# ETH3D/badslam

Hardware: NVIDIA H100
Metric: surfel_keyframe_residuals_per_second_per_BA_iteration (higher is better)
Workload: dtype f32

## Files before the change

badslam_b200/csrc/handle.hpp:

```cpp
#pragma once

#include <cuda_runtime.h>

#include <algorithm>
#include <atomic>
#include <condition_variable>
#include <cstdio>
#include <cstdlib>
#include <map>
#include <mutex>
#include <string>
#include <thread>
#include <vector>

#include "../../include/badba.h"
#include "host_math.hpp"
#include "kernels.cuh"
#include "odometry.cuh"

namespace bba {

template <class R, auto Free>
struct Owned {
  R r{};
// ... 115 lines not shown
  float depth_a = 0.f;
  int cf_w = 0, cf_h = 0;
  int sm_count = 132;
  std::mutex error_mu;
  std::map<std::thread::id, std::string> errors;

  float* surfels = nullptr;
  size_t surfel_pitch_bytes = 0;
  uint32_t surfels_size = 0;
  uint8_t* active = nullptr;
  bba::DeviceBuffer<float> owned_surfels;
  size_t owned_surfel_pitch = 0;
  bba::DeviceBuffer<uint8_t> owned_active;

  bba::DeviceBuffer<float> d_cfactor;
  std::vector<bba::Keyframe> keyframes;
  bba::DeviceBuffer<bba::KfDevice> d_kfs;

  struct Staging {
    bba::PinnedBuffer<bba::KfDevice> h_kfs;
    bba::Event event;
    bool pending = false;
    bba::LumaStaging luma;
    bba::PitchedBuffer color;
    bba::Texture scratch;
  } staging;

  struct PoseStep {
    bba::DeviceBuffer<bba::KfDevice> d_work_records;
    bba::DeviceBuffer<float> d_pose_est;
    bba::DeviceBuffer<double> d_acc;
    bba::DeviceBuffer<unsigned long long> d_stage_counts;
    bba::DeviceBuffer<int> d_work[2];
    bba::DeviceBuffer<int> d_count;
    bba::DeviceBuffer<int> d_iterations;
    bba::DeviceBuffer<int> d_converged;
    bba::DeviceBuffer<double> d_first_stats;
    bba::DeviceBuffer<unsigned long long> d_totals;
    bba::DeviceBuffer<unsigned int> d_queue;
    bba::MappedBuffer<int> flag;
    volatile int* h_flag = nullptr;
    int* d_flag = nullptr;
    bba::PinnedBuffer<float> h_pose_est;
    bba::PinnedBuffer<int> h_work;
    bba::PinnedBuffer<int> h_iterations;
    bba::PinnedBuffer<int> h_converged;
    bba::PinnedBuffer<double> h_first_stats;
    bba::PinnedBuffer<unsigned long long> h_totals;
    struct Order {
      bba::DeviceBuffer<uint32_t> words;
      bba::DeviceBuffer<unsigned char> temp;
      bba::DeviceBuffer<float> stream;
      bba::DeviceBuffer<float> boxes;
      bba::SpatialOrderBuffers view{};
      uint32_t capacity = 0;
    } order;
    uint32_t order_n = 0;
    bool order_stale = true;
  } pose;

  struct Geometry {
    bba::DeviceBuffer<int> d_list;
    bba::PinnedBuffer<int> h_list;
    bba::DeviceBuffer<unsigned int> d_queue;
    bba::DeviceBuffer<unsigned int> d_tile_epoch;
    const uint32_t* perm = nullptr;
    bba::DeviceBuffer<float> d_intr;
    bba::DeviceBuffer<double> d_intr_sums;
    bba::DeviceBuffer<int> d_all_list;
    bba::PinnedBuffer<double> h_intr_sums;
    bba::PinnedBuffer<float> h_intr_x1;
  } geo;

  struct Lifecycle {
    bba::DeviceBuffer<unsigned int> d_sup;
    bba::DeviceBuffer<unsigned int> d_cell_bits;
    bba::DeviceBuffer<unsigned int> d_flags;
    bba::DeviceBuffer<unsigned int> d_scan_out;
    bba::DeviceBuffer<unsigned int> d_scan_sums;
    bba::DeviceBuffer<bba::CovisEntry> d_covis;
    bba::PinnedBuffer<bba::CovisEntry> h_covis;
    bba::DeviceBuffer<bba::KfRadius> d_kf_radius;
    bba::PinnedBuffer<bba::KfRadius> h_kf_radius;
    bba::DeviceBuffer<unsigned int> d_deleted_count;
    bba::PinnedBuffer<unsigned int> h_deleted_count;
    bba::DeviceBuffer<unsigned int> d_compact_sums;
  } life;
  int last_ba_iteration_count = -1;

  struct Pcg {
    bba::DeviceBuffer<float> d_vec[5];
    bba::DeviceBuffer<double> d_scalars;
    bba::PinnedBuffer<double> h_scalars;
    bba::PinnedBuffer<float> h_delta;
  } pcg;

  struct Exchange {
    bba_collective_fn collective = nullptr;
    void* collective_user = nullptr;
    bba::DeviceBuffer<float> d_exchange;
    bba::DeviceBuffer<float> d_pose_pack;
    bba::PinnedBuffer<float> h_pose_pack;
    bba::DeviceBuffer<int> d_local_ids;
    bba::DeviceBuffer<float> d_count_xchg;
    bba::PinnedBuffer<float> h_count_xchg;
    bba::DeviceBuffer<float> d_barrier;
// ... 139 lines not shown
```

badslam_b200/csrc/kernels.cu:

```cuda
#include "persistent.cuh"

#include <cuda.h>

#include <algorithm>

namespace bba {


__device__ __forceinline__ uint32_t SmemAddr(const void* p) { return static_cast<uint32_t>(__cvta_generic_to_shared(p)); }

__device__ __forceinline__ void MbarInit(uint64_t* bar, uint32_t count) {
  asm volatile("mbarrier.init.shared::cta.b64 [%0], %1;" ::"r"(SmemAddr(bar)), "r"(count));
}
__device__ __forceinline__ void FenceBarrierInit() { asm volatile("fence.mbarrier_init.release.cluster;" ::: "memory"); }
__device__ __forceinline__ void MbarArriveExpectTx(uint64_t* bar, uint32_t bytes) {
  asm volatile("mbarrier.arrive.expect_tx.shared::cta.b64 _, [%0], %1;" ::"r"(SmemAddr(bar)), "r"(bytes) : "memory");
}
__device__ __forceinline__ void MbarArrive(uint64_t* bar) {
  asm volatile("mbarrier.arrive.shared::cta.b64 _, [%0];" ::"r"(SmemAddr(bar)) : "memory");
}
__device__ __forceinline__ void MbarWait(uint64_t* bar, uint32_t parity) {
  asm volatile(
      "{\n"
      ".reg .pred p;\n"
      "WAIT_LOOP:\n"
      "mbarrier.try_wait.parity.shared::cta.b64 p, [%0], %1;\n"
      "@p bra.uni WAIT_DONE;\n"
      "bra.uni WAIT_LOOP;\n"
      "WAIT_DONE:\n"
      "}\n" ::"r"(SmemAddr(bar)),
      "r"(parity)
      : "memory");
}
__device__ __forceinline__ bool MbarTest(uint64_t* bar, uint32_t parity) {
  uint32_t done;
  asm volatile(
      "{\n"
      ".reg .pred p;\n"
      "mbarrier.test_wait.parity.shared::cta.b64 p, [%1], %2;\n"
      "selp.u32 %0, 1, 0, p;\n"
      "}\n"
      : "=r"(done)
      : "r"(SmemAddr(bar)), "r"(parity)
      : "memory");
  return done != 0;
}
__device__ __forceinline__ void BulkCopyG2S(void* smem_dst, const void* gmem_src, uint32_t bytes, uint64_t* bar) {
  asm volatile("cp.async.bulk.shared::cluster.global.mbarrier::complete_tx::bytes [%0], [%1], %2, [%3];" ::"r"(SmemAddr(smem_dst)),
               "l"(gmem_src), "r"(bytes), "r"(SmemAddr(bar))
               : "memory");
}


__device__ __forceinline__ cudaTextureObject_t UniformTexture(cudaTextureObject_t tex) {
  const unsigned long long t = tex;
  const unsigned lo = __shfl_sync(0xffffffffu, static_cast<unsigned>(t), 0);
  const unsigned hi = __shfl_sync(0xffffffffu, static_cast<unsigned>(t >> 32), 0);
  return (static_cast<unsigned long long>(hi) << 32) | lo;
}

constexpr int kPoseMinCtas = 2;
constexpr int kPoseChunkShift = 8;
constexpr int kPoseThreads = 256;
constexpr int kPoseUnroll = 1;
constexpr int kPoseStagedRows = 7;
constexpr int kPoseStagedRowsPre = 14;
static_assert(kPoseStagedRowsPre == kPoseStreamRows, "the PRE instantiations stage every row of the pose stream");
constexpr int kPoseGroup = 8;

__device__ __forceinline__ bool CornersOutsideView(const CameraParams& cam, const float* __restrict__ T, float px, float py, float pz) {
  float v[3], a[3];
#pragma unroll
  for (int r = 0; r < 3; ++r) {
    v[r] = T[4 * r] * px + T[4 * r + 1] * py + T[4 * r + 2] * pz + T[4 * r + 3];
    a[r] = fabsf(T[4 * r] * px) + fabsf(T[4 * r + 1] * py) + fabsf(T[4 * r + 2] * pz) + fabsf(T[4 * r + 3]);
  }
  constexpr float e = 1e-5f;
  const float l_x = cam.cx + 1.f, r_x = cam.cx - static_cast<float>(cam.w) - 1.f;
  const float l_y = cam.cy + 1.f, r_y = cam.cy - static_cast<float>(cam.h) - 1.f;
  unsigned out = (v[2] < -e * a[2]) ? 1u : 0u;
  out |= (cam.fx * v[0] + l_x * v[2] < -e * (cam.fx * a[0] + fabsf(l_x) * a[2])) ? 2u : 0u;
  out |= (cam.fx * v[0] + r_x * v[2] > e * (cam.fx * a[0] + fabsf(r_x) * a[2])) ? 4u : 0u;
  out |= (cam.fy * v[1] + l_y * v[2] < -e * (cam.fy * a[1] + fabsf(l_y) * a[2])) ? 8u : 0u;
  out |= (cam.fy * v[1] + r_y * v[2] > e * (cam.fy * a[1] + fabsf(r_y) * a[2])) ? 16u : 0u;
  if (!(cam.fx > 0.f && cam.fy > 0.f)) out &= 1u;
  return __reduce_and_sync(0xffffffffu, out) != 0u;
}
__device__ __forceinline__ bool BoxOutsideView(const CameraParams& cam, const float* __restrict__ T, const float* box, int lane) {
  const int c = lane & 7;
  return CornersOutsideView(cam, T, box[(c & 1) ? 4 : 0], box[(c & 2) ? 5 : 1], box[(c & 4) ? 6 : 2]);
}

constexpr int kPoseProducerWarps = 8;
constexpr int kPoseConsumerWarps = 4;
constexpr int kPoseWsThreads = 32 * (kPoseProducerWarps + kPoseConsumerWarps);
constexpr int kPoseProducerRegs = 72;
constexpr int kPoseConsumerRegs = 96;
static_assert(kPoseProducerWarps * kPoseProducerRegs + kPoseConsumerWarps * kPoseConsumerRegs ==
                  (kPoseProducerWarps + kPoseConsumerWarps) * 80, "register split");
constexpr int kPoseRecFields = 16;
constexpr int kPoseRingSlots = 2;
constexpr int kPoseBatchFloats = kPoseRecFields * 32;
constexpr size_t kPoseRingBytes = sizeof(float) * kPoseBatchFloats * kPoseRingSlots * kPoseProducerWarps;

template <int N>
__device__ __forceinline__ void SetMaxRegsDec() { asm volatile("setmaxnreg.dec.sync.aligned.u32 %0;\n" ::"n"(N)); }
template <int N>
__device__ __forceinline__ void SetMaxRegsInc() { asm volatile("setmaxnreg.inc.sync.aligned.u32 %0;\n" ::"n"(N)); }

template <bool STATS>
__device__ __forceinline__ void AccumulatePair(const CameraParams& cam, const Assoc& r, const DescEval& e, bool photo,
                                               float (&acc)[kPoseAccSize]) {
  acc[27] += 1.f;
  if (cam.use_depth) {
    float inv_stddev;
    Vec3 up;
    const float raw = DepthResidual(cam, r, &inv_stddev, &up);
    float J[6];
    DepthPoseJacobian(r, inv_stddev, up, J);
    AccumulateHb(acc, J, raw, DepthWeight(raw));
    if (STATS) acc[29] += DepthCost(raw);
  }
  if (cam.use_desc && photo) {
    acc[28] += 1.f;
    float J[6];
    DescPoseJacobian(cam, r.lp, e.gx1, e.gy1, J);
    AccumulateHb(acc, J, e.r1, DescWeight(e.r1));
    DescPoseJacobian(cam, r.lp, e.gx2, e.gy2, J);
    AccumulateHb(acc, J, e.r2, DescWeight(e.r2));
    if (STATS) {
      acc[30] += DescCost(e.r1);
      acc[31] += DescCost(e.r2);
    }
  }
}

template <bool STATS>
__device__ __forceinline__ void AccumulateRecord(const CameraParams& cam, const float* rec, float (&acc)[kPoseAccSize]) {
  Assoc r;
  r.lp = V3(rec[0 * 32], rec[1 * 32], rec[2 * 32]);
  r.ln = V3(rec[3 * 32], rec[4 * 32], rec[5 * 32]);
  r.d = rec[6 * 32];
  r.nx = rec[7 * 32];
  r.ny = rec[8 * 32];
  DescEval e;
  e.r1 = rec[9 * 32];
  e.r2 = rec[10 * 32];
  e.gx1 = rec[11 * 32];
  e.gy1 = rec[12 * 32];
  e.gx2 = rec[13 * 32];
  e.gy2 = rec[14 * 32];
  AccumulatePair<STATS>(cam, r, e, rec[15 * 32] != 0.f, acc);
}

template <int TILE, bool STATS, bool PRE>
__global__ void __launch_bounds__(PRE ? kPoseWsThreads : kPoseThreads, kPoseMinCtas)
    PoseAccumulateKernel(const __grid_constant__ PoseAccumulateArgs args) {
  constexpr int kRows = PRE ? kPoseStagedRowsPre : kPoseStagedRows;
  extern __shared__ __align__(128) unsigned char smem_raw[];
  float* stage_base = reinterpret_cast<float*>(smem_raw);
  float* rings = stage_base + 2 * kRows * TILE;
  __shared__ __align__(16) KfDevice s_kf[2][kPoseGroup];
  __shared__ __align__(16) float s_box[2][PRE ? TILE / kSpatialChunk : 1][8];
  __shared__ __align__(8) uint64_t full_bar[2];
  __shared__ unsigned int s_item[2];
  __shared__ int s_sub[2];
  __shared__ __align__(8) uint64_t batch_full[PRE ? kPoseProducerWarps : 1][kPoseRingSlots];
  __shared__ __align__(8) uint64_t batch_empty[PRE ? kPoseProducerWarps : 1][kPoseRingSlots];
  __shared__ int3 batch_hdr[PRE ? kPoseProducerWarps : 1][kPoseRingSlots];

  const int n_work = __ldg(args.work_count);
  if (n_work <= 0) return;

  const int tid = threadIdx.x;
  const int lane = tid & 31;
  const int warp = tid >> 5;
  const uint32_t n_tiles = (args.n + TILE - 1) / TILE;
  const uint32_t n_groups = (n_work + kPoseGroup - 1) / kPoseGroup;
  const uint32_t n_items = n_groups * n_tiles;
  constexpr int kTileShift = (TILE == 1024) ? 10 : (TILE == 512) ? 9 : 8;

  const CameraParams& cam = args.cam;
  constexpr int kRowIds[kPoseStagedRows] = {kRowX, kRowY, kRowZ, kRowNormal, kRowRadiusSq, kRowD1, kRowD2};

  auto issue_tile = [&](uint32_t item, int s) {
    const uint32_t group = item / n_tiles, tile = item - group * n_tiles;
    const uint32_t base = tile * TILE;
    const uint32_t cnt = min(static_cast<uint32_t>(TILE), args.n - base);
    const uint32_t bytes = ((cnt * 4u + 15u) / 16u) * 16u;
    const uint32_t kf_bytes = static_cast<uint32_t>(sizeof(KfDevice)) * min(kPoseGroup, n_work - static_cast<int>(group) * kPoseGroup);
    const uint32_t box_bytes = PRE ? (cnt + kSpatialChunk - 1) / kSpatialChunk * 8 * sizeof(float) : 0u;
    MbarArriveExpectTx(&full_bar[s], bytes * kRows + kf_bytes + box_bytes);
    BulkCopyG2S(&s_kf[s][0], args.work_records + static_cast<size_t>(group) * kPoseGroup, kf_bytes, &full_bar[s]);
    if (PRE) {
      BulkCopyG2S(&s_box[s][0][0], args.boxes + static_cast<size_t>(base / kSpatialChunk) * 8, box_bytes, &full_bar[s]);
#pragma unroll
      for (int r = 0; r < kPoseStreamRows; ++r)
        BulkCopyG2S(stage_base + (s * kRows + r) * TILE, args.stream + static_cast<size_t>(r) * args.stream_pitch + base, bytes,
                    &full_bar[s]);
    } else {
#pragma unroll
      for (int r = 0; r < kPoseStagedRows; ++r) {
        BulkCopyG2S(stage_base + (s * kRows + r) * TILE,
                    args.surfels + static_cast<size_t>(kRowIds[r]) * args.pitch + base, bytes, &full_bar[s]);
      }
    }
  };

  __shared__ int s_done[2];
  constexpr int kWarps = PRE ? kPoseProducerWarps : kPoseThreads / 32;
  auto arm_stage = [&](int s) {
    s_sub[s] = 0;
    s_done[s] = 0;
    const unsigned int item = atomicAdd(args.queue, 1u);
    s_item[s] = item;
    if (item < n_items) issue_tile(item, s);
    else MbarArrive(&full_bar[s]);
  };
  if (tid == 0) {
    MbarInit(&full_bar[0], 1);
    MbarInit(&full_bar[1], 1);
    if (PRE) {
      for (int p = 0; p < kPoseProducerWarps; ++p)
        for (int b = 0; b < kPoseRingSlots; ++b) {
          MbarInit(&batch_full[p][b], 32);
          MbarInit(&batch_empty[p][b], 32);
        }
    }
    FenceBarrierInit();
    arm_stage(0);
    arm_stage(1);
  }
  __syncthreads();

  uint32_t batch_seq = 0;
  bool batch_owned = false;
  int batch_fill = 0;
  if constexpr (PRE) {
    if (warp >= kPoseProducerWarps) {
      SetMaxRegsInc<kPoseConsumerRegs>();
      const int c = warp - kPoseProducerWarps;
      float acc0[kPoseAccSize], acc1[kPoseAccSize];
#pragma unroll
      for (int i = 0; i < kPoseAccSize; ++i) acc0[i] = acc1[i] = 0.f;
      uint32_t seq0 = 0, seq1 = 0;
      bool done0 = false, done1 = false;
      auto consume = [&](int p, uint32_t& seq, bool& done, float (&acc)[kPoseAccSize]) {
        const int b = seq & 1;
        if (!__all_sync(0xffffffffu, MbarTest(&batch_full[p][b], (seq >> 1) & 1))) return false;
        const int3 h = batch_hdr[p][b];
        if (h.z < 0) {
          done = true;
          return true;
        }
        if (lane < h.x) AccumulateRecord<STATS>(args.cam, rings + (p * kPoseRingSlots + b) * kPoseBatchFloats + lane, acc);
        MbarArrive(&batch_empty[p][b]);
        ++seq;
        if (h.y) {
          const float total = WarpTransposeReduce(acc, lane);
          atomicAdd(args.acc + static_cast<size_t>(h.z) * kPoseAccSize + lane, static_cast<double>(total));
#pragma unroll
          for (int i = 0; i < kPoseAccSize; ++i) acc[i] = 0.f;
        }
        return true;
      };
      while (!(done0 && done1)) {
        bool progress = false;
        if (!done0) progress |= consume(c, seq0, done0, acc0);
        if (!done1) progress |= consume(c + kPoseConsumerWarps, seq1, done1, acc1);
        if (!progress) __nanosleep(32);
      }
      return;
    }
    SetMaxRegsDec<kPoseProducerRegs>();
  }
  float* my_ring = rings + warp * kPoseRingSlots * kPoseBatchFloats;
  auto acquire_slot = [&](uint32_t u) {
    MbarWait(&batch_empty[warp][u & 1], ((u >> 1) & 1) ^ 1);
  };
  auto commit_slot = [&](uint32_t u, int pairs, bool last, int kf) {
    if (lane == 0) batch_hdr[warp][u & 1] = make_int3(pairs, last ? 1 : 0, kf);
    MbarArrive(&batch_full[warp][u & 1]);
  };

  for (uint32_t it = 0;; ++it) {
    const int s = it & 1;
    MbarWait(&full_bar[s], (it >> 1) & 1);
    const unsigned int item = *reinterpret_cast<volatile unsigned int*>(&s_item[s]);
    if (item >= n_items) break;

    const float* sx = stage_base + (s * kRows + 0) * TILE;
    const float* sy = sx + TILE;
    const float* sz = sy + TILE;
    const float* sn = sz + TILE;
    const float* sr = sn + TILE;
    const float* sd1 = PRE ? sz + TILE : sr + TILE;
    const float* sd2 = sd1 + TILE;
    const float* sf = sd2 + TILE;
    const uint32_t group = item / n_tiles;
    const uint32_t tile = item - group * n_tiles;
    const uint32_t base = tile * TILE;
    const uint32_t cnt = min(static_cast<uint32_t>(TILE), args.n - base);
    const int kfs_in_group = min(kPoseGroup, n_work - static_cast<int>(group) * kPoseGroup);
    const int wanted_shift = n_work >= 4 ? kPoseChunkShift : 7;
    const int chunk_shift = wanted_shift < kTileShift ? wanted_shift : kTileShift;
    const uint32_t chunk_len = 1u << chunk_shift;
    const int chunks_per_tile = TILE >> chunk_shift;
    const int n_sub = kfs_in_group * chunks_per_tile;

    for (;;) {
      int sub = 0;
      if (lane == 0) sub = atomicAdd(&s_sub[s], 1);
      sub = __shfl_sync(0xffffffffu, sub, 0);
      if (sub >= n_sub) break;
      const int kf_local = sub / chunks_per_tile;
      const uint32_t j0 = static_cast<uint32_t>(sub - kf_local * chunks_per_tile) << chunk_shift;
      if (j0 >= cnt) continue;
      const uint32_t j1 = min(cnt, j0 + chunk_len);
      KfRegs K;
      const int kf = LoadKfShared(&s_kf[s][kf_local], &K);
      if (PRE && BoxOutsideView(cam, K.T, s_box[s][PRE ? j0 / kSpatialChunk : 0], lane)) continue;
      K.tex = UniformTexture(K.tex);

      float acc[kPoseAccSize];
#pragma unroll
      for (int i = 0; i < kPoseAccSize; ++i) acc[i] = 0.f;
      unsigned touched = 0;
      unsigned n_inimg = 0, n_depthok = 0;

#pragma unroll kPoseUnroll
      for (uint32_t j = j0 + lane; j < j0 + (j1 - j0 + 31u) / 32u * 32u; j += 32) {
        int st = 0;
        Assoc r;
        Vec3 gp, nrm;
        DescEval e;
        bool photo = false;
        if (j < j1) {
          gp = V3(sx[j], sy[j], sz[j]);
          if (ProjectIntoImage(cam, K.T, gp, &r)) {
            const PixelLoads l = LoadPixel(cam, K.depth, K.depth_pitch, K.normals, K.normals_pitch, r);
            nrm = PRE ? V3(sf[j], sf[TILE + j], sf[2 * TILE + j]) : UnpackNormal(__float_as_uint(sn[j]));
            if (cam.use_desc) {
              float ccx, ccy;
              photo = DepthToColor(cam, r.pxf, r.pyf, &ccx, &ccy);
              float t1x, t1y, t2x, t2y;
              if (PRE) {
                ProjectTangentPoints(cam, K.T, V3(sf[3 * TILE + j], sf[4 * TILE + j], sf[5 * TILE + j]),
                                     V3(sf[6 * TILE + j], sf[7 * TILE + j], sf[8 * TILE + j]), &t1x, &t1y, &t2x, &t2y);
              } else {
                TangentProjections(cam, K.T, gp, nrm, sr[j], &t1x, &t1y, &t2x, &t2y);
              }
              EvalDescriptor(K.tex, ccx, ccy, t1x, t1y, t2x, t2y, sd1[j], sd2[j], &e);
            }
            st = Associate(cam, K.T, nrm, l, &r);
          }
        }
        if (STATS) {
          n_inimg += st >= 1;
          n_depthok += st >= 2;
        }
        const unsigned assoc_mask = __ballot_sync(0xffffffffu, st == 3);
        if (assoc_mask == 0) continue;
        touched |= assoc_mask;
        if constexpr (PRE) {
          const int m = __popc(assoc_mask);
          const int pos = batch_fill + __popc(assoc_mask & ((1u << lane) - 1u));
          const bool spill = batch_fill + m > 32;
          if (!batch_owned) acquire_slot(batch_seq);
          batch_owned = true;
          if (spill) acquire_slot(batch_seq + 1);
          if (st == 3) {
            float* rec = my_ring + ((batch_seq + (pos >> 5)) & 1) * kPoseBatchFloats + (pos & 31);
            rec[0 * 32] = r.lp.x; rec[1 * 32] = r.lp.y; rec[2 * 32] = r.lp.z;
            rec[3 * 32] = r.ln.x; rec[4 * 32] = r.ln.y; rec[5 * 32] = r.ln.z;
// ... 10 lines not shown
            batch_fill += m;
          }
        } else if (st == 3) {
          AccumulatePair<STATS>(cam, r, e, photo, acc);
        }
      }

      if (PRE && touched) {
        commit_slot(batch_seq, batch_fill, true, kf);
        ++batch_seq;
        batch_owned = false;
        batch_fill = 0;
      } else if (touched) {
        const float total = WarpTransposeReduce(acc, lane);
        atomicAdd(args.acc + static_cast<size_t>(kf) * kPoseAccSize + lane, static_cast<double>(total));
      }
      if (STATS) {
        n_inimg = __reduce_add_sync(0xffffffffu, n_inimg);
        n_depthok = __reduce_add_sync(0xffffffffu, n_depthok);
      }
      if (STATS && lane == 0 && n_inimg) {
        atomicAdd(args.stage_counts + 2 * kf, static_cast<unsigned long long>(n_inimg));
        if (n_depthok) atomicAdd(args.stage_counts + 2 * kf + 1, static_cast<unsigned long long>(n_depthok));
      }
    }
    __syncwarp();
    if (lane == 0) {
      __threadfence_block();
      if (atomicAdd(&s_done[s], 1) == kWarps - 1) {
        __threadfence_block();
        arm_stage(s);
      }
    }
  }
  if (PRE) {
    if (!batch_owned) acquire_slot(batch_seq);
    commit_slot(batch_seq, 0, false, -1);
  }
}

__global__ void __launch_bounds__(128) PackWorkRecordsKernel(const KfDevice* __restrict__ kfs, const int* __restrict__ work_list,
                                                             const int* __restrict__ work_count, KfDevice* __restrict__ records) {
  const int n = __ldg(work_count);
  constexpr int kWords = sizeof(KfDevice) / 16;
  for (int i = blockIdx.x * blockDim.x + threadIdx.x; i < n * kWords; i += gridDim.x * blockDim.x) {
    const int rec = i / kWords, w = i - rec * kWords;
    const int kf = __ldg(work_list + rec);
    uint4 v = __ldg(reinterpret_cast<const uint4*>(kfs + kf) + w);
    if (w == kWords - 1) v.y = static_cast<unsigned int>(kf);
    reinterpret_cast<uint4*>(records + rec)[w] = v;
  }
}

template <int TILE, bool STATS, bool PRE>
static void LaunchPoseAccumulateT(const PoseAccumulateArgs& args, int sm_count, cudaStream_t stream) {
  const size_t smem = static_cast<size_t>(2) * (PRE ? kPoseStagedRowsPre : kPoseStagedRows) * TILE * sizeof(float) + (PRE ? kPoseRingBytes : 0);
  static bool configured = false;
  if (!configured) {
    cudaFuncSetAttribute(PoseAccumulateKernel<TILE, STATS, PRE>, cudaFuncAttributeMaxDynamicSharedMemorySize, static_cast<int>(smem));
    configured = true;
  }
  PoseAccumulateKernel<TILE, STATS, PRE><<<kPoseMinCtas * sm_count, PRE ? kPoseWsThreads : kPoseThreads, smem, stream>>>(args);
}

template <bool STATS>
static void LaunchPoseAccumulateS(const PoseAccumulateArgs& args, int sm_count, int variant, cudaStream_t stream) {
  if (variant == kPoseVariantAuto) {
    const uint64_t slots = static_cast<uint64_t>(kPoseMinCtas * sm_count) * 4;
    if (args.stream != nullptr) variant = args.n >= slots * 512 ? kPoseVariant512Pre : kPoseVariant256Pre;
    else variant = args.n >= slots * 1024 ? kPoseVariant1024 : args.n >= slots * 512 ? kPoseVariant512 : kPoseVariant256;
  }
  switch (variant) {
    case kPoseVariant256Pre: LaunchPoseAccumulateT<256, STATS, true>(args, sm_count, stream); break;
    case kPoseVariant512Pre: LaunchPoseAccumulateT<512, STATS, true>(args, sm_count, stream); break;
    case kPoseVariant256: LaunchPoseAccumulateT<256, STATS, false>(args, sm_count, stream); break;
    case kPoseVariant512: LaunchPoseAccumulateT<512, STATS, false>(args, sm_count, stream); break;
    case kPoseVariant1024: LaunchPoseAccumulateT<1024, STATS, false>(args, sm_count, stream); break;
  }
}

void LaunchPoseAccumulate(const PoseAccumulateArgs& args, int sm_count, bool with_stats, int max_work, cudaStream_t stream, int variant) {
  if (args.n == 0) return;
  PackWorkRecordsKernel<<<(max_work * 6 + 127) / 128, 128, 0, stream>>>(args.kfs, args.work_list, args.work_count, args.work_records);
  if (with_stats) LaunchPoseAccumulateS<true>(args, sm_count, variant, stream);
  else LaunchPoseAccumulateS<false>(args, sm_count, variant, stream);
}


constexpr int kGeoThreads = 256;
constexpr int kGeoGroup = 32;

__device__ __forceinline__ void StageGroupRecords(const KfDevice* __restrict__ kfs, const int* __restrict__ kf_list, int count,
                                                  KfDevice* dst, int lane) {
  constexpr int kWords = sizeof(KfDevice) / 16;
  __syncwarp();
  const int my_kf = lane < count ? __ldg(kf_list + lane) : 0;
#pragma unroll
  for (int w = 0; w < (kGeoGroup * kWords + 31) / 32; ++w) {
    const int idx = w * 32 + lane, rec = idx / kWords, part = idx - rec * kWords;
    const int kf = __shfl_sync(0xffffffffu, my_kf, rec & 31);
    if (rec < count) {
      uint4 v = __ldg(reinterpret_cast<const uint4*>(kfs + kf) + part);
      reinterpret_cast<uint4*>(dst + rec)[part] = v;
    }
  }
  __syncwarp();
}

__device__ __forceinline__ void WarpBoxCorner(const Vec3& p, bool in, int lane, float* cx, float* cy, float* cz) {
  const float c[3] = {p.x, p.y, p.z};
  float corner[3];
#pragma unroll
  for (int ax = 0; ax < 3; ++ax) {
    const bool f = in && isfinite(c[ax]);
    const unsigned int lo = __reduce_min_sync(0xffffffffu, f ? OrderedBits(c[ax]) : 0xffffffffu);
    const unsigned int hi = __reduce_max_sync(0xffffffffu, f ? OrderedBits(c[ax]) : 0u);
    corner[ax] = FromOrderedBits(((lane >> ax) & 1) ? hi : lo);
  }
  *cx = corner[0];
  *cy = corner[1];
  *cz = corner[2];
}

__device__ __forceinline__ void StoreSurfelRow(const GeometryArgs& a, int row, uint32_t i, float v) {
  StoreReplicas(a.surfels, a.peers.surfels, a.peers.count, static_cast<size_t>(row) * a.pitch + i, v);
}

template <bool DETERMINE, bool NORMALS>
__global__ void __launch_bounds__(kGeoThreads) ActivationNormalsKernel(const __grid_constant__ GeometryArgs a) {
  extern __shared__ __align__(16) unsigned char geo_smem[];
  KfDevice* s_kfs = reinterpret_cast<KfDevice*>(geo_smem);
  const uint32_t tile_len = 1u << a.tile_shift;
  const uint32_t n_tiles = (a.end - a.begin + tile_len - 1) >> a.tile_shift;
  const uint32_t n_groups = (a.kf_count + kGeoGroup - 1) / kGeoGroup;
  const uint32_t n_items = n_groups * n_tiles;
  const size_t P = a.pitch, F = a.stream_pitch;
  const int lane = threadIdx.x & 31;
  uint32_t group, tile;
// ... 356 lines not shown
```

badslam_b200/csrc/kernels.cuh:

```cuda
#pragma once

#include <cuda_runtime.h>
#include <stdint.h>

#include "device_math.cuh"

namespace bba {

constexpr int kPoseAccSize = 32;

struct PoseAccumulateArgs {
  CameraParams cam;
  const float* surfels;
  uint32_t pitch;
  uint32_t n;
  const KfDevice* kfs;
  const int* work_list;
  const int* work_count;
  const float* stream;
  uint32_t stream_pitch;
  const float* boxes;
  KfDevice* work_records;
  double* acc;
  unsigned long long* stage_counts;
  unsigned int* queue;
};

constexpr int kSpatialChunk = 256;
struct SpatialOrderBuffers {
  uint32_t* keys_in;
  uint32_t* keys_out;
  uint32_t* index_in;
  uint32_t* perm;
  unsigned int* bounds;
  void* temp;
  size_t temp_bytes;
};
size_t SpatialOrderTempBytes(uint32_t capacity);
void LaunchSpatialOrder(const float* surfels, uint32_t pitch, uint32_t n, const SpatialOrderBuffers& b, cudaStream_t stream);
constexpr int kPoseStreamRows = 14;
void LaunchPoseStream(const float* surfels, uint32_t pitch, uint32_t n, const uint32_t* perm, float* stream, uint32_t stream_pitch,
                      float* boxes, cudaStream_t cuda_stream);
enum PoseVariant { kPoseVariantAuto = 0, kPoseVariant256Pre = 1, kPoseVariant512Pre = 2, kPoseVariant256 = 3, kPoseVariant512 = 4,
                   kPoseVariant1024 = 5 };
inline bool PoseVariantValid(int v) { return v >= kPoseVariantAuto && v <= kPoseVariant1024; }
inline bool PoseVariantPre(int v) { return v == kPoseVariant256Pre || v == kPoseVariant512Pre; }
void LaunchPoseAccumulate(const PoseAccumulateArgs& args, int sm_count, bool with_stats, int max_work, cudaStream_t stream,
                          int variant = kPoseVariantAuto);

struct PoseSolveArgs {
  KfDevice* kfs;
  float* pose_est;
  double* acc;
  unsigned long long* stage_counts;
  const int* work_in;
  const int* count_in;
  int* work_out;
  int* count_out;
  int* iterations;
  int* converged;
  double* first_stats;
  unsigned long long* totals;
  volatile int* host_flag;
  unsigned int* queue;
  int iteration;
  int max_iterations;
};
void LaunchPoseSolve(const PoseSolveArgs& args, cudaStream_t stream);

constexpr int kMaxPeers = 7;
struct PeerSet {
  int count;
  float* surfels[kMaxPeers];
  uint8_t* active[kMaxPeers];
};

struct GeometryArgs {
  CameraParams cam;
  float* surfels;
  uint32_t pitch;
  uint32_t n;
  uint32_t begin, end;
  uint32_t shard_rank, shard_world;
  const uint32_t* perm;
  float* stream;
  uint32_t stream_pitch;
  uint8_t* active;
  const KfDevice* kfs;
  const int* kf_list;
  int kf_count;
  unsigned int* queue;
  unsigned int* tile_epoch;
  int tile_shift;
  PeerSet peers;
};
constexpr int kGeoStreamRows = 8;
static_assert(kGeoStreamRows <= kPoseStreamRows, "the geometry stream lives in the pose stream's buffer");
void LaunchGeometryStream(const GeometryArgs& args, bool desc_rows, cudaStream_t stream);
int LaunchActivationAndNormals(const GeometryArgs& args, int sm_count, bool determine_activation, bool update_normals, cudaStream_t stream);
int LaunchPositionAndDescriptor(const GeometryArgs& args, int sm_count, cudaStream_t stream);
// ... 145 lines not shown
```

badslam_b200/csrc/pose_step.cu:

```cuda
#include <cstring>
#include <thread>

#include "handle.hpp"

namespace bba {

bba_status EnsureSpatialOrder(bba_handle h, bool sort, bool rebuild, cudaStream_t s) {
  auto& p = h->pose;
  const uint32_t n = h->surfels_size;
  if (n > p.order.capacity) {
    p.order = {};
    p.order_stale = true;
    const uint32_t cap = (n + 511u) / 512u * 512u;
    const size_t sort_bytes = SpatialOrderTempBytes(cap);
    BBA_CUDA(h, p.order.words.Reserve(4 * static_cast<size_t>(cap) + 8));
    BBA_CUDA(h, p.order.temp.Reserve(sort_bytes));
    BBA_CUDA(h, p.order.stream.Reserve(kPoseStreamRows * static_cast<size_t>(cap)));
    BBA_CUDA(h, p.order.boxes.Reserve(8 * static_cast<size_t>(cap / kSpatialChunk)));
    uint32_t* words = p.order.words;
    p.order.view.keys_in = words;
    p.order.view.keys_out = words + cap;
    p.order.view.index_in = words + 2 * static_cast<size_t>(cap);
    p.order.view.perm = words + 3 * static_cast<size_t>(cap);
    p.order.view.bounds = words + 4 * static_cast<size_t>(cap);
    p.order.view.temp = p.order.temp;
    p.order.view.temp_bytes = sort_bytes;
    p.order.capacity = cap;
  }
  if (sort && (rebuild || p.order_stale || p.order_n != n)) {
    LaunchSpatialOrder(h->surfels, static_cast<uint32_t>(h->surfel_pitch_bytes / sizeof(float)), n, p.order.view, s);
    BBA_CUDA(h, cudaGetLastError());
    h->launches += 3;
    p.order_n = n;
    p.order_stale = false;
  }
  return BBA_OK;
}

namespace {

bba_status PreparePoseAccumulate(bba_handle h, int n_work, int variant, cudaStream_t s, PoseAccumulateArgs* acc) {
  auto& p = h->pose;
  SetSurfelFields(h, acc);
  acc->kfs = h->d_kfs;
  acc->work_records = p.d_work_records;
  acc->acc = p.d_acc;
  acc->stage_counts = p.d_stage_counts;
  acc->queue = p.d_queue;
  acc->stream = nullptr;
  acc->stream_pitch = 0;
  acc->boxes = nullptr;
  const bool pre = variant == kPoseVariantAuto ? h->cfg.use_descriptor_residuals && n_work >= 4 : PoseVariantPre(variant);
  if (pre && h->surfels_size > 0) {
    const bool sort = variant != kPoseVariantAuto ||
                      static_cast<uint64_t>(h->surfels_size) * static_cast<uint64_t>(n_work) >= kSpatialOrderMinPairs;
    if (bba_status st = EnsureSpatialOrder(h, sort, false, s)) return st;
    LaunchPoseStream(h->surfels, acc->pitch, h->surfels_size, sort ? p.order.view.perm : nullptr, p.order.stream,
                     p.order.capacity, p.order.boxes, s);
    ++h->launches;
    acc->stream = p.order.stream;
    acc->stream_pitch = p.order.capacity;
    acc->boxes = p.order.boxes;
  }
  return BBA_OK;
}

bba_status StagePoseWork(bba_handle h, const std::vector<int>& ids, const std::vector<Pose>& poses, const int* owner, cudaStream_t s,
                         int* n_work) {
  auto& p = h->pose;
  const int K = static_cast<int>(h->keyframes.size()), M = h->cfg.max_keyframes;
  if (bba_status st = WaitStaging(h)) return st;
  for (int k = 0; k < K; ++k) FillKfDevice(h->keyframes[k], h->keyframes[k].pose, h->staging.h_kfs + k);
  int n = 0;
  for (size_t i = 0; i < ids.size(); ++i) {
    FillKfDevice(h->keyframes[ids[i]], poses[i], h->staging.h_kfs + ids[i]);
    if (!owner || owner[i] == h->cfg.rank) p.h_work[n++] = ids[i];
  }
  p.h_work[M] = n;
  p.h_work[M + 1] = 0;
  BBA_CUDA(h, cudaMemcpyAsync(h->d_kfs, h->staging.h_kfs, sizeof(KfDevice) * K, cudaMemcpyHostToDevice, s));
  if (n) BBA_CUDA(h, cudaMemcpyAsync(p.d_work[0], p.h_work, sizeof(int) * n, cudaMemcpyHostToDevice, s));
  BBA_CUDA(h, cudaMemcpyAsync(p.d_count, p.h_work + M, sizeof(int) * 2, cudaMemcpyHostToDevice, s));
  BBA_CUDA(h, cudaMemsetAsync(p.d_acc, 0, sizeof(double) * kPoseAccSize * K, s));
  BBA_CUDA(h, cudaMemsetAsync(p.d_stage_counts, 0, sizeof(unsigned long long) * 2 * K, s));
  BBA_CUDA(h, cudaMemsetAsync(p.d_queue, 0, sizeof(unsigned int), s));
  *n_work = n;
  return BBA_OK;
}

bba_status PoseCoeffsBatch(bba_handle h, const std::vector<int>& ids, const std::vector<Pose>& poses, int variant, bool with_stats,
                           cudaStream_t s, std::vector<double>* rec, std::vector<unsigned long long>* sc) {
  auto& p = h->pose;
  const int K = static_cast<int>(h->keyframes.size());
  int count = 0;
  if (bba_status st = StagePoseWork(h, ids, poses, nullptr, s, &count)) return st;
  PoseAccumulateArgs acc;
  if (bba_status st = PreparePoseAccumulate(h, count, variant, s, &acc)) return st;
  acc.work_list = p.d_work[0];
  acc.work_count = p.d_count;
  if (h->surfels_size > 0) {
    LaunchPoseAccumulate(acc, h->sm_count, with_stats, count, s, variant);
    h->launches += 2;
  }
  BBA_CUDA(h, cudaGetLastError());
  rec->resize(static_cast<size_t>(kPoseAccSize) * K);
  sc->resize(2 * static_cast<size_t>(K));
  BBA_CUDA(h, cudaMemcpyAsync(rec->data(), p.d_acc, sizeof(double) * rec->size(), cudaMemcpyDeviceToHost, s));
  BBA_CUDA(h, cudaMemcpyAsync(sc->data(), p.d_stage_counts, sizeof(unsigned long long) * sc->size(), cudaMemcpyDeviceToHost, s));
  BBA_CUDA(h, cudaMemsetAsync(p.d_acc, 0, sizeof(double) * rec->size(), s));
  BBA_CUDA(h, cudaMemsetAsync(p.d_stage_counts, 0, sizeof(unsigned long long) * sc->size(), s));
  BBA_CUDA(h, cudaStreamSynchronize(s));
  h->staging.pending = false;
  return BBA_OK;
}

void FramePoseResult(bba_handle h, int id, float out[7], int* iterations, int* converged) {
  std::memcpy(out, h->pose.h_pose_est + 7 * id, sizeof(float) * 7);
  if (iterations) *iterations = h->pose.h_iterations[id];
  if (converged) *converged = h->pose.h_converged[id];
}

}

bba_status RunPoseStep(bba_handle h, const std::vector<int>& ids, const std::vector<Pose>& init, int max_iterations, cudaStream_t s) {
  auto& p = h->pose;
  auto& x = h->xchg;
  const int K = static_cast<int>(h->keyframes.size());
  const int n = static_cast<int>(ids.size());
  if (n == 0) return BBA_OK;
  const int world = h->cfg.world_size;
  if (bba_status st = CheckCollective(h)) return st;
  std::vector<int> owner(n, 0);
  if (world > 1) AssignKeyframes(h, ids, &owner);
  int n_local = 0;
  if (bba_status st = StagePoseWork(h, ids, init, owner.data(), s, &n_local)) return st;
  for (int k = 0; k < K; ++k) PoseToArray(h->keyframes[k].pose, p.h_pose_est + 7 * k);
  for (int i = 0; i < n; ++i) PoseToArray(init[i], p.h_pose_est + 7 * ids[i]);
  BBA_CUDA(h, cudaMemcpyAsync(p.d_pose_est, p.h_pose_est, sizeof(float) * 7 * K, cudaMemcpyHostToDevice, s));
  if (world > 1 && n_local) BBA_CUDA(h, cudaMemcpyAsync(x.d_local_ids, p.h_work, sizeof(int) * n_local, cudaMemcpyHostToDevice, s));
  BBA_CUDA(h, cudaMemsetAsync(p.d_iterations, 0, sizeof(int) * K, s));
  BBA_CUDA(h, cudaMemsetAsync(p.d_converged, 0, sizeof(int) * K, s));
  if (bba_status st = MarkStaging(h, s)) return st;

  PoseAccumulateArgs acc;
  if (bba_status st = PreparePoseAccumulate(h, n_local, kPoseVariantAuto, s, &acc)) return st;
  PoseSolveArgs sol;
  sol.kfs = h->d_kfs;
  sol.pose_est = p.d_pose_est;
  sol.acc = p.d_acc;
  sol.stage_counts = p.d_stage_counts;
  sol.iterations = p.d_iterations;
  sol.converged = p.d_converged;
  sol.first_stats = p.d_first_stats;
  sol.max_iterations = max_iterations;
  sol.totals = p.d_totals;
  sol.host_flag = p.d_flag;
  sol.queue = p.d_queue;
  p.h_flag[0] = 0;
  p.h_flag[1] = n_local;
  if (h->profiling) BBA_CUDA(h, cudaMemsetAsync(p.d_totals, 0, sizeof(unsigned long long) * 8, s));
  int enqueued = 0;
  for (int it = 0; it < max_iterations; ++it) {
    const int cur = it & 1;
    acc.work_list = p.d_work[cur];
    acc.work_count = p.d_count + cur;
    if (h->surfels_size > 0) {
      if (h->profiling && it < 32) BBA_CUDA(h, cudaEventRecord(h->prof_ev[2 * it], s));
      LaunchPoseAccumulate(acc, h->sm_count, it == 0 || h->profiling >= 2, n_local, s);
      if (h->profiling && it < 32) BBA_CUDA(h, cudaEventRecord(h->prof_ev[2 * it + 1], s));
      h->launches += 2;
    }
    sol.work_in = p.d_work[cur];
    sol.count_in = p.d_count + cur;
    sol.work_out = p.d_work[cur ^ 1];
    sol.count_out = p.d_count + (cur ^ 1);
    sol.iteration = it;
    LaunchPoseSolve(sol, s);
    ++h->launches;
    ++enqueued;
    constexpr int kDepth = 3;
    if (it >= kDepth) {
      unsigned int polls = 0;
      while (p.h_flag[0] < it - kDepth + 1) {
        if (cudaStreamQuery(s) != cudaErrorNotReady) break;
        if (++polls > 256 && (polls & 15) == 0) std::this_thread::yield();
      }
    }
    if (it >= 1 && p.h_flag[0] >= 1 && p.h_flag[1] == 0) break;
  }
  BBA_CUDA(h, cudaGetLastError());
  if (world > 1) {
    BBA_CUDA(h, cudaMemsetAsync(x.d_pose_pack, 0, sizeof(float) * kPoseSlot * K, s));
    LaunchPackPoseResults(x.d_local_ids, n_local, p.d_pose_est, p.d_iterations, p.d_converged, p.d_first_stats, x.d_pose_pack, s);
    ++h->launches;
    x.collective(x.collective_user, BBA_COLLECTIVE_ALLREDUCE_SUM, x.d_pose_pack, static_cast<size_t>(kPoseSlot) * K, s);
    x.replicated_pass_pending = false;
    BBA_CUDA(h, cudaMemcpyAsync(x.h_pose_pack, x.d_pose_pack, sizeof(float) * kPoseSlot * K, cudaMemcpyDeviceToHost, s));
  } else {
    BBA_CUDA(h, cudaMemcpyAsync(p.h_pose_est, p.d_pose_est, sizeof(float) * 7 * K, cudaMemcpyDeviceToHost, s));
    BBA_CUDA(h, cudaMemcpyAsync(p.h_iterations, p.d_iterations, sizeof(int) * K, cudaMemcpyDeviceToHost, s));
    BBA_CUDA(h, cudaMemcpyAsync(p.h_converged, p.d_converged, sizeof(int) * K, cudaMemcpyDeviceToHost, s));
    BBA_CUDA(h, cudaMemcpyAsync(p.h_first_stats, p.d_first_stats, sizeof(double) * 8 * K, cudaMemcpyDeviceToHost, s));
  }
  if (h->profiling) BBA_CUDA(h, cudaMemcpyAsync(p.h_totals, p.d_totals, sizeof(unsigned long long) * 8, cudaMemcpyDeviceToHost, s));
  BBA_CUDA(h, cudaStreamSynchronize(s));
  h->staging.pending = false;
  if (world > 1) {
    for (int i = 0; i < n; ++i) {
      const int kf = ids[i];
      const float* slot = x.h_pose_pack + static_cast<size_t>(kf) * kPoseSlot;
      std::memcpy(p.h_pose_est + 7 * kf, slot, sizeof(float) * 7);
      p.h_iterations[kf] = static_cast<int>(slot[7] + 0.5f);
      p.h_converged[kf] = static_cast<int>(slot[8] + 0.5f);
      for (int j = 0; j < 8; ++j) p.h_first_stats[8 * kf + j] = slot[9 + j];
    }
  }
  if (h->kf_cost.size() < static_cast<size_t>(K)) h->kf_cost.resize(h->cfg.max_keyframes, 0.f);
  for (int kf : ids)
    h->kf_cost[kf] = static_cast<float>(std::max(1, p.h_iterations[kf]) * (0.06 * h->surfels_size + p.h_first_stats[8 * kf + 5]));
  if (h->profiling && h->surfels_size > 0) {
    int real_iterations = 0;
    for (int i = 0; i < n_local; ++i) real_iterations = std::max(real_iterations, p.h_iterations[p.h_work[i]]);
    for (int it = 0; it < std::min(real_iterations, std::min(enqueued, 32)); ++it) {
// ... 124 lines not shown
```

Baseline: 22.92 billion.

## Precompute per-item visibility masks and skip empty work items in pose accumulation

Measured after the change: 22.77 billion (median of 6 runs). About the same (-0.7%).

```diff
diff --git a/badslam_b200/csrc/handle.hpp b/badslam_b200/csrc/handle.hpp
--- a/badslam_b200/csrc/handle.hpp
+++ b/badslam_b200/csrc/handle.hpp
@@ -191,6 +191,7 @@
       bba::DeviceBuffer<unsigned char> temp;
       bba::DeviceBuffer<float> stream;
       bba::DeviceBuffer<float> boxes;
+      bba::DeviceBuffer<bba::PoseMask> masks;
       bba::SpatialOrderBuffers view{};
       uint32_t capacity = 0;
     } order;
diff --git a/badslam_b200/csrc/kernels.cu b/badslam_b200/csrc/kernels.cu
--- a/badslam_b200/csrc/kernels.cu
+++ b/badslam_b200/csrc/kernels.cu
@@ -68,7 +68,13 @@
 static_assert(kPoseStagedRowsPre == kPoseStreamRows, "the PRE instantiations stage every row of the pose stream");
 constexpr int kPoseGroup = 8;
 
-__device__ __forceinline__ bool CornersOutsideView(const CameraParams& cam, const float* __restrict__ T, float px, float py, float pz) {
+__device__ __forceinline__ int PoseChunkShift(int n_work, int tile_shift) {
+  const int wanted_shift = n_work >= 4 ? kPoseChunkShift : 7;
+  return wanted_shift < tile_shift ? wanted_shift : tile_shift;
+}
+
+__device__ __forceinline__ unsigned CornerOutsidePlanes(const CameraParams& cam, const float* __restrict__ T, float px, float py,
+                                                        float pz) {
   float v[3], a[3];
 #pragma unroll
   for (int r = 0; r < 3; ++r) {
@@ -84,11 +90,37 @@
   out |= (cam.fy * v[1] + l_y * v[2] < -e * (cam.fy * a[1] + fabsf(l_y) * a[2])) ? 8u : 0u;
   out |= (cam.fy * v[1] + r_y * v[2] > e * (cam.fy * a[1] + fabsf(r_y) * a[2])) ? 16u : 0u;
   if (!(cam.fx > 0.f && cam.fy > 0.f)) out &= 1u;
-  return __reduce_and_sync(0xffffffffu, out) != 0u;
-}
-__device__ __forceinline__ bool BoxOutsideView(const CameraParams& cam, const float* __restrict__ T, const float* box, int lane) {
-  const int c = lane & 7;
-  return CornersOutsideView(cam, T, box[(c & 1) ? 4 : 0], box[(c & 2) ? 5 : 1], box[(c & 4) ? 6 : 2]);
+  return out;
+}
+__device__ __forceinline__ bool CornersOutsideView(const CameraParams& cam, const float* __restrict__ T, float px, float py, float pz) {
+  return __reduce_and_sync(0xffffffffu, CornerOutsidePlanes(cam, T, px, py, pz)) != 0u;
+}
+__device__ __forceinline__ unsigned BoxCornerOutsidePlanes(const CameraParams& cam, const float* __restrict__ T, const float* box, int c) {
+  return CornerOutsidePlanes(cam, T, box[(c & 1) ? 4 : 0], box[(c & 2) ? 5 : 1], box[(c & 4) ? 6 : 2]);
+}
+
+__device__ __forceinline__ int NthSetBit(uint32_t m, int n) {
+  int pos = 0;
+#pragma unroll
+  for (int w = 16; w >= 1; w >>= 1) {
+    const int c = __popc((m >> pos) & ((1u << w) - 1u));
+    if (n >= c) {
+      n -= c;
+      pos += w;
+    }
+  }
+  return pos;
+}
+__device__ __forceinline__ int NthSetBit(unsigned long long m, int n) {
+  const uint32_t lo = static_cast<uint32_t>(m);
+  const int c = __popc(lo);
+  return n < c ? NthSetBit(lo, n) : 32 + NthSetBit(static_cast<uint32_t>(m >> 32), n - c);
+}
+__device__ __forceinline__ int PopCount(uint32_t m) { return __popc(m); }
+__device__ __forceinline__ int PopCount(unsigned long long m) { return __popcll(m); }
+__device__ __forceinline__ uint32_t WarpOr(uint32_t m) { return __reduce_or_sync(0xffffffffu, m); }
+__device__ __forceinline__ unsigned long long WarpOr(unsigned long long m) {
+  return (static_cast<unsigned long long>(WarpOr(static_cast<uint32_t>(m >> 32))) << 32) | WarpOr(static_cast<uint32_t>(m));
 }
 
 constexpr int kPoseProducerWarps = 8;
@@ -157,13 +189,14 @@
 __global__ void __launch_bounds__(PRE ? kPoseWsThreads : kPoseThreads, kPoseMinCtas)
     PoseAccumulateKernel(const __grid_constant__ PoseAccumulateArgs args) {
   constexpr int kRows = PRE ? kPoseStagedRowsPre : kPoseStagedRows;
+  constexpr int kGroup = PRE ? kPoseGroupPre : kPoseGroup;
   extern __shared__ __align__(128) unsigned char smem_raw[];
   float* stage_base = reinterpret_cast<float*>(smem_raw);
   float* rings = stage_base + 2 * kRows * TILE;
-  __shared__ __align__(16) KfDevice s_kf[2][kPoseGroup];
-  __shared__ __align__(16) float s_box[2][PRE ? TILE / kSpatialChunk : 1][8];
+  __shared__ __align__(16) KfDevice s_kf[2][kGroup];
   __shared__ __align__(8) uint64_t full_bar[2];
   __shared__ unsigned int s_item[2];
+  __shared__ PoseMask s_mask[2];
   __shared__ int s_sub[2];
   __shared__ __align__(8) uint64_t batch_full[PRE ? kPoseProducerWarps : 1][kPoseRingSlots];
   __shared__ __align__(8) uint64_t batch_empty[PRE ? kPoseProducerWarps : 1][kPoseRingSlots];
@@ -176,7 +209,7 @@
   const int lane = tid & 31;
   const int warp = tid >> 5;
   const uint32_t n_tiles = (args.n + TILE - 1) / TILE;
-  const uint32_t n_groups = (n_work + kPoseGroup - 1) / kPoseGroup;
+  const uint32_t n_groups = (n_work + kGroup - 1) / kGroup;
   const uint32_t n_items = n_groups * n_tiles;
   constexpr int kTileShift = (TILE == 1024) ? 10 : (TILE == 512) ? 9 : 8;
 
@@ -188,12 +221,10 @@
     const uint32_t base = tile * TILE;
     const uint32_t cnt = min(static_cast<uint32_t>(TILE), args.n - base);
     const uint32_t bytes = ((cnt * 4u + 15u) / 16u) * 16u;
-    const uint32_t kf_bytes = static_cast<uint32_t>(sizeof(KfDevice)) * min(kPoseGroup, n_work - static_cast<int>(group) * kPoseGroup);
-    const uint32_t box_bytes = PRE ? (cnt + kSpatialChunk - 1) / kSpatialChunk * 8 * sizeof(float) : 0u;
-    MbarArriveExpectTx(&full_bar[s], bytes * kRows + kf_bytes + box_bytes);
-    BulkCopyG2S(&s_kf[s][0], args.work_records + static_cast<size_t>(group) * kPoseGroup, kf_bytes, &full_bar[s]);
+    const uint32_t kf_bytes = static_cast<uint32_t>(sizeof(KfDevice)) * min(kGroup, n_work - static_cast<int>(group) * kGroup);
+    MbarArriveExpectTx(&full_bar[s], bytes * kRows + kf_bytes);
+    BulkCopyG2S(&s_kf[s][0], args.work_records + static_cast<size_t>(group) * kGroup, kf_bytes, &full_bar[s]);
     if (PRE) {
-      BulkCopyG2S(&s_box[s][0][0], args.boxes + static_cast<size_t>(base / kSpatialChunk) * 8, box_bytes, &full_bar[s]);
 #pragma unroll
       for (int r = 0; r < kPoseStreamRows; ++r)
         BulkCopyG2S(stage_base + (s * kRows + r) * TILE, args.stream + static_cast<size_t>(r) * args.stream_pitch + base, bytes,
@@ -212,7 +243,10 @@
   auto arm_stage = [&](int s) {
     s_sub[s] = 0;
     s_done[s] = 0;
-    const unsigned int item = atomicAdd(args.queue, 1u);
+    unsigned int item = atomicAdd(args.queue, 1u);
+    if constexpr (PRE) {
+      while (item < n_items && (s_mask[s] = __ldg(args.masks + item)) == 0) item = atomicAdd(args.queue, 1u);
+    }
     s_item[s] = item;
     if (item < n_items) issue_tile(item, s);
     else MbarArrive(&full_bar[s]);
@@ -301,16 +335,21 @@
     const uint32_t tile = item - group * n_tiles;
     const uint32_t base = tile * TILE;
     const uint32_t cnt = min(static_cast<uint32_t>(TILE), args.n - base);
-    const int kfs_in_group = min(kPoseGroup, n_work - static_cast<int>(group) * kPoseGroup);
-    const int wanted_shift = n_work >= 4 ? kPoseChunkShift : 7;
-    const int chunk_shift = wanted_shift < kTileShift ? wanted_shift : kTileShift;
+    const int kfs_in_group = min(kGroup, n_work - static_cast<int>(group) * kGroup);
+    const int chunk_shift = PoseChunkShift(n_work, kTileShift);
     const uint32_t chunk_len = 1u << chunk_shift;
     const int chunks_per_tile = TILE >> chunk_shift;
     const int n_sub = kfs_in_group * chunks_per_tile;
 
     for (;;) {
       int sub = 0;
-      if (lane == 0) sub = atomicAdd(&s_sub[s], 1);
+      if (lane == 0) {
+        sub = atomicAdd(&s_sub[s], 1);
+        if (PRE) {
+          const PoseMask live = *reinterpret_cast<volatile PoseMask*>(&s_mask[s]);
+          sub = sub < PopCount(live) ? NthSetBit(live, sub) : n_sub;
+        }
+      }
       sub = __shfl_sync(0xffffffffu, sub, 0);
       if (sub >= n_sub) break;
       const int kf_local = sub / chunks_per_tile;
@@ -319,7 +358,6 @@
       const uint32_t j1 = min(cnt, j0 + chunk_len);
       KfRegs K;
       const int kf = LoadKfShared(&s_kf[s][kf_local], &K);
-      if (PRE && BoxOutsideView(cam, K.T, s_box[s][PRE ? j0 / kSpatialChunk : 0], lane)) continue;
       K.tex = UniformTexture(K.tex);
 
       float acc[kPoseAccSize];
@@ -436,38 +474,89 @@
   }
 }
 
+__global__ void __launch_bounds__(256) PoseVisibilityKernel(const CameraParams cam, const KfDevice* __restrict__ records,
+                                                            const int* __restrict__ work_count, const float* __restrict__ boxes,
+                                                            uint32_t n, int tile_shift, PoseMask* __restrict__ masks) {
+  const int n_work = __ldg(work_count);
+  if (n_work <= 0) return;
+  const uint32_t n_tiles = (n + (1u << tile_shift) - 1) >> tile_shift;
+  const uint32_t n_items = static_cast<uint32_t>((n_work + kPoseGroupPre - 1) / kPoseGroupPre) * n_tiles;
+  const int chunk_shift = PoseChunkShift(n_work, tile_shift);
+  const int chunks_per_tile = 1 << (tile_shift - chunk_shift);
+  const int boxes_per_tile = 1 << (tile_shift - 8);
+  const int chunks_per_box = 1 << (8 - chunk_shift);
+  static_assert(kSpatialChunk == 256, "box and chunk indexing");
+  const int lane = threadIdx.x & 31, corner = lane & 7;
+  const uint32_t warps = gridDim.x * (blockDim.x >> 5);
+  for (uint32_t item = blockIdx.x * (blockDim.x >> 5) + (threadIdx.x >> 5); item < n_items; item += warps) {
+    const uint32_t group = item / n_tiles, tile = item - group * n_tiles;
+    const uint32_t base = tile << tile_shift;
+    const uint32_t cnt = min(1u << tile_shift, n - base);
+    const int n_tests = min(kPoseGroupPre, n_work - static_cast<int>(group) * kPoseGroupPre) * boxes_per_tile;
+    PoseMask mask = 0;
+    for (int t0 = 0; t0 < n_tests; t0 += 4) {
+      const int t = t0 + (lane >> 3);
+      const int slot = t / boxes_per_tile, b = t - slot * boxes_per_tile;
+      const bool tested = t < n_tests && (static_cast<uint32_t>(b) << 8) < cnt;
+      unsigned out = 0;
+      if (tested) {
+        out = BoxCornerOutsidePlanes(cam, records[group * kPoseGroupPre + slot].T, boxes + (static_cast<size_t>(base >> 8) + b) * 8,
+                                     corner);
+      }
+      out &= __shfl_xor_sync(0xffffffffu, out, 1);
+      out &= __shfl_xor_sync(0xffffffffu, out, 2);
+      out &= __shfl_xor_sync(0xffffffffu, out, 4);
+      const uint32_t j0 = (static_cast<uint32_t>(b) << 8) + (static_cast<uint32_t>(corner) << chunk_shift);
+      if (tested && out == 0u && corner < chunks_per_box && j0 < cnt)
+        mask |= PoseMask(1) << (slot * chunks_per_tile + b * chunks_per_box + corner);
+    }
+    mask = WarpOr(mask);
+    if (lane == 0) masks[item] = mask;
+  }
+}
+
 template <int TILE, bool STATS, bool PRE>
-static void LaunchPoseAccumulateT(const PoseAccumulateArgs& args, int sm_count, cudaStream_t stream) {
+static void LaunchPoseAccumulateT(const PoseAccumulateArgs& args, int sm_count, int max_work, cudaStream_t stream) {
   const size_t smem = static_cast<size_t>(2) * (PRE ? kPoseStagedRowsPre : kPoseStagedRows) * TILE * sizeof(float) + (PRE ? kPoseRingBytes : 0);
   static bool configured = false;
   if (!configured) {
     cudaFuncSetAttribute(PoseAccumulateKernel<TILE, STATS, PRE>, cudaFuncAttributeMaxDynamicSharedMemorySize, static_cast<int>(smem));
     configured = true;
   }
+  if constexpr (PRE) {
+    static_assert(TILE == 256 || TILE == 512, "PRE tiles");
+    constexpr int kTileShift = (TILE == 512) ? 9 : 8;
+    const uint32_t n_tiles = (args.n + TILE - 1) / TILE;
+    const uint64_t items = static_cast<uint64_t>((max_work + kPoseGroupPre - 1) / kPoseGroupPre) * n_tiles;
+    const int blocks = static_cast<int>(std::min<uint64_t>((items + 7) / 8, static_cast<uint64_t>(8) * sm_count));
+    PoseVisibilityKernel<<<std::max(blocks, 1), 256, 0, stream>>>(args.cam, args.work_records, args.work_count, args.boxes, args.n,
+                                                                   kTileShift, args.masks);
+  }
   PoseAccumulateKernel<TILE, STATS, PRE><<<kPoseMinCtas * sm_count, PRE ? kPoseWsThreads : kPoseThreads, smem, stream>>>(args);
 }
 
 template <bool STATS>
-static void LaunchPoseAccumulateS(const PoseAccumulateArgs& args, int sm_count, int variant, cudaStream_t stream) {
+static int LaunchPoseAccumulateS(const PoseAccumulateArgs& args, int sm_count, int max_work, int variant, cudaStream_t stream) {
   if (variant == kPoseVariantAuto) {
     const uint64_t slots = static_cast<uint64_t>(kPoseMinCtas * sm_count) * 4;
     if (args.stream != nullptr) variant = args.n >= slots * 512 ? kPoseVariant512Pre : kPoseVariant256Pre;
     else variant = args.n >= slots * 1024 ? kPoseVariant1024 : args.n >= slots * 512 ? kPoseVariant512 : kPoseVariant256;
   }
   switch (variant) {
-    case kPoseVariant256Pre: LaunchPoseAccumulateT<256, STATS, true>(args, sm_count, stream); break;
-    case kPoseVariant512Pre: LaunchPoseAccumulateT<512, STATS, true>(args, sm_count, stream); break;
-    case kPoseVariant256: LaunchPoseAccumulateT<256, STATS, false>(args, sm_count, stream); break;
-    case kPoseVariant512: LaunchPoseAccumulateT<512, STATS, false>(args, sm_count, stream); break;
-    case kPoseVariant1024: LaunchPoseAccumulateT<1024, STATS, false>(args, sm_count, stream); break;
-  }
-}
-
-void LaunchPoseAccumulate(const PoseAccumulateArgs& args, int sm_count, bool with_stats, int max_work, cudaStream_t stream, int variant) {
-  if (args.n == 0) return;
+    case kPoseVariant256Pre: LaunchPoseAccumulateT<256, STATS, true>(args, sm_count, max_work, stream); break;
+    case kPoseVariant512Pre: LaunchPoseAccumulateT<512, STATS, true>(args, sm_count, max_work, stream); break;
+    case kPoseVariant256: LaunchPoseAccumulateT<256, STATS, false>(args, sm_count, max_work, stream); break;
+    case kPoseVariant512: LaunchPoseAccumulateT<512, STATS, false>(args, sm_count, max_work, stream); break;
+    case kPoseVariant1024: LaunchPoseAccumulateT<1024, STATS, false>(args, sm_count, max_work, stream); break;
+  }
+  return PoseVariantPre(variant) ? 3 : 2;
+}
+
+int LaunchPoseAccumulate(const PoseAccumulateArgs& args, int sm_count, bool with_stats, int max_work, cudaStream_t stream, int variant) {
+  if (args.n == 0) return 0;
   PackWorkRecordsKernel<<<(max_work * 6 + 127) / 128, 128, 0, stream>>>(args.kfs, args.work_list, args.work_count, args.work_records);
-  if (with_stats) LaunchPoseAccumulateS<true>(args, sm_count, variant, stream);
-  else LaunchPoseAccumulateS<false>(args, sm_count, variant, stream);
+  return with_stats ? LaunchPoseAccumulateS<true>(args, sm_count, max_work, variant, stream)
+                    : LaunchPoseAccumulateS<false>(args, sm_count, max_work, variant, stream);
 }
 
 
diff --git a/badslam_b200/csrc/kernels.cuh b/badslam_b200/csrc/kernels.cuh
--- a/badslam_b200/csrc/kernels.cuh
+++ b/badslam_b200/csrc/kernels.cuh
@@ -3,11 +3,20 @@
 #include <cuda_runtime.h>
 #include <stdint.h>
 
+#include <type_traits>
+
 #include "device_math.cuh"
 
 namespace bba {
 
 constexpr int kPoseAccSize = 32;
+
+constexpr int kPoseGroupPre = 16;
+using PoseMask = std::conditional_t<(2 * kPoseGroupPre > 32), unsigned long long, uint32_t>;
+static_assert(2 * kPoseGroupPre <= 8 * static_cast<int>(sizeof(PoseMask)), "a work item's sub-items fit its mask");
+inline size_t PoseMaskCount(int max_work, uint32_t capacity) {
+  return static_cast<size_t>((max_work + kPoseGroupPre - 1) / kPoseGroupPre) * ((capacity + 255u) / 256u);
+}
 
 struct PoseAccumulateArgs {
   CameraParams cam;
@@ -20,6 +29,7 @@
   const float* stream;
   uint32_t stream_pitch;
   const float* boxes;
+  PoseMask* masks;
   KfDevice* work_records;
   double* acc;
   unsigned long long* stage_counts;
@@ -45,7 +55,7 @@
                    kPoseVariant1024 = 5 };
 inline bool PoseVariantValid(int v) { return v >= kPoseVariantAuto && v <= kPoseVariant1024; }
 inline bool PoseVariantPre(int v) { return v == kPoseVariant256Pre || v == kPoseVariant512Pre; }
-void LaunchPoseAccumulate(const PoseAccumulateArgs& args, int sm_count, bool with_stats, int max_work, cudaStream_t stream,
+int LaunchPoseAccumulate(const PoseAccumulateArgs& args, int sm_count, bool with_stats, int max_work, cudaStream_t stream,
                           int variant = kPoseVariantAuto);
 
 struct PoseSolveArgs {
diff --git a/badslam_b200/csrc/pose_step.cu b/badslam_b200/csrc/pose_step.cu
--- a/badslam_b200/csrc/pose_step.cu
+++ b/badslam_b200/csrc/pose_step.cu
@@ -17,6 +17,7 @@
     BBA_CUDA(h, p.order.temp.Reserve(sort_bytes));
     BBA_CUDA(h, p.order.stream.Reserve(kPoseStreamRows * static_cast<size_t>(cap)));
     BBA_CUDA(h, p.order.boxes.Reserve(8 * static_cast<size_t>(cap / kSpatialChunk)));
+    BBA_CUDA(h, p.order.masks.Reserve(PoseMaskCount(h->cfg.max_keyframes, cap)));
     uint32_t* words = p.order.words;
     p.order.view.keys_in = words;
     p.order.view.keys_out = words + cap;
@@ -50,6 +51,7 @@
   acc->stream = nullptr;
   acc->stream_pitch = 0;
   acc->boxes = nullptr;
+  acc->masks = nullptr;
   const bool pre = variant == kPoseVariantAuto ? h->cfg.use_descriptor_residuals && n_work >= 4 : PoseVariantPre(variant);
   if (pre && h->surfels_size > 0) {
     const bool sort = variant != kPoseVariantAuto ||
@@ -61,6 +63,7 @@
     acc->stream = p.order.stream;
     acc->stream_pitch = p.order.capacity;
     acc->boxes = p.order.boxes;
+    acc->masks = p.order.masks;
   }
   return BBA_OK;
 }
@@ -98,10 +101,7 @@
   if (bba_status st = PreparePoseAccumulate(h, count, variant, s, &acc)) return st;
   acc.work_list = p.d_work[0];
   acc.work_count = p.d_count;
-  if (h->surfels_size > 0) {
-    LaunchPoseAccumulate(acc, h->sm_count, with_stats, count, s, variant);
-    h->launches += 2;
-  }
+  if (h->surfels_size > 0) h->launches += LaunchPoseAccumulate(acc, h->sm_count, with_stats, count, s, variant);
   BBA_CUDA(h, cudaGetLastError());
   rec->resize(static_cast<size_t>(kPoseAccSize) * K);
   sc->resize(2 * static_cast<size_t>(K));
@@ -166,9 +166,8 @@
     acc.work_count = p.d_count + cur;
     if (h->surfels_size > 0) {
       if (h->profiling && it < 32) BBA_CUDA(h, cudaEventRecord(h->prof_ev[2 * it], s));
-      LaunchPoseAccumulate(acc, h->sm_count, it == 0 || h->profiling >= 2, n_local, s);
+      h->launches += LaunchPoseAccumulate(acc, h->sm_count, it == 0 || h->profiling >= 2, n_local, s);
       if (h->profiling && it < 32) BBA_CUDA(h, cudaEventRecord(h->prof_ev[2 * it + 1], s));
-      h->launches += 2;
     }
     sol.work_in = p.d_work[cur];
     sol.count_in = p.d_count + cur;
```
